# tuffy/libdvd-audio

Measured on AMD Instinct MI355X. Metric: decoded PCM Msamples/s (bit-exact) on 6ch/96k/24b MLP, higher is better.
Workload: dtype int32 (int64 accumulate)

## Files before the change

### libdvd-audio_amd/csrc/mlp_decode.h

```cpp
#pragma once
#include <hip/hip_runtime.h>
#if defined(__HIP_DEVICE_COMPILE__) && !defined(__gfx950__)
#error "mlp_decode.h is written for gfx950 (MI355X): hand-placed s_waitcnt encodings and gfx950 inline asm"
#endif
#include <stdint.h>
#include <type_traits>
#include "mlp_bounds.h"
#include "mlp_index.h"
#include "mlp_tables.h"

namespace mlp {

constexpr int DEC_THREADS = 128;
constexpr int DEC_WAVES = DEC_THREADS / 64;
constexpr int MAXCH = 8;
constexpr int MAXMAT = 6;
constexpr int RING_PLANES = 8;
constexpr int RING_DWORDS = RING_PLANES * 4;
constexpr int CHUNK_DWORDS = 16;
constexpr int OUT_ROWS = 4;
constexpr uint32_t YIELD_LONELY = 48;
#ifndef DVDA_HDR_GATE_TURNS
#define DVDA_HDR_GATE_TURNS 32
#endif
// ... 128 lines not shown
    const uint64_t *out_stride;
    uint32_t *seg_status;
    uint32_t *seg_rows;
    int32_t *iir_ws;
    uint32_t *mat_ws;
    uint32_t total_lanes;
    unsigned long long *dbg;
    int32_t *fir_ws;
    int32_t *fb;
    const int32_t *init_fir;
    DecodeSummary *summary;
    uint32_t interleaved;
    uint32_t wav_bits;
    uint32_t coop_min_seg;
    const uint32_t *hetero;
    const uint32_t *lane_seg;
    const uint32_t *cls;
    uint32_t only_S;
    uint32_t *seg_meta;
    uint32_t *yield_req;
    const uint32_t *seg_check;
    const uint32_t *list;
    uint32_t list_base, list_n;
    const uint32_t *list_n_ptr;
    const uint4 *plan;
    int32_t *res;
    uint32_t *brec;
    uint32_t *frec;
    WsCaps caps;
    uint32_t coop;
    struct CoopState *coop_state;
    struct CoopResult *coop_result;
    uint32_t coop_spare;
};

constexpr uint32_t COOP_MAX_SEG = 4096;
constexpr uint32_t COOP_MAX_AU = 32768;
__device__ __forceinline__ bool coop_takes(const DecodeArgs &a)
{
    if (a.coop)
        return a.coop == 64u;
    uint32_t n_seg = *a.n_seg_ptr;
    if (n_seg > a.max_seg)
        n_seg = a.max_seg;
    return n_seg <= COOP_MAX_SEG && a.seg_fbase[n_seg] <= COOP_MAX_AU;
}



__device__ __forceinline__ int32_t mask_q(int32_t x, uint32_t q)
{
    return (int32_t)((uint32_t)x & (0xFFFFFFFFu << q));
}
__device__ __forceinline__ uint32_t nib(uint32_t pack, uint32_t i) { return (pack >> (4 * i)) & 0xFu; }
__device__ __forceinline__ int32_t lo16(uint32_t v) { return (int32_t)(v << 16) >> 16; }
__device__ __forceinline__ int32_t hi16(uint32_t v) { return (int32_t)v >> 16; }

__device__ __forceinline__ int32_t huff_center(uint32_t codebook, uint32_t lb)
{
    if (codebook) {
        const int ss = (int)lb + 2 - (int)codebook;
        return 7 * (1 << lb) + (ss >= 0 ? (1 << ss) : 0);
    }
    const int ss = (int)lb - 1;
    return ss >= 0 ? (1 << ss) : 0;
}

__device__ __forceinline__ uint32_t be32(uint32_t v) { return __builtin_bswap32(v); }
template <int RD = RING_DWORDS>
__device__ __forceinline__ void ring_store16(uint32_t *dst, const uint4 &a, const uint4 &b, const uint4 &c,
                                             const uint4 &d, bool first_plane)
{
    const uint32_t a0 = be32(a.x);
    uint32_t *const e = dst - 15 * 64;
    if (first_plane)
        dst[-RD * 64] = a0;
    e[15 * 64] = a0;         e[14 * 64] = be32(a.y); e[13 * 64] = be32(a.z); e[12 * 64] = be32(a.w);
    e[11 * 64] = be32(b.x);  e[10 * 64] = be32(b.y); e[9 * 64] = be32(b.z);  e[8 * 64] = be32(b.w);
    e[7 * 64] = be32(c.x);   e[6 * 64] = be32(c.y);  e[5 * 64] = be32(c.z);  e[4 * 64] = be32(c.w);
    e[3 * 64] = be32(d.x);   e[2 * 64] = be32(d.y);  e[1 * 64] = be32(d.z);  e[0 * 64] = be32(d.w);
}

template <int RD>
__device__ __forceinline__ void ring_store4(uint32_t *dst, const uint4 &a, bool first_plane)
{
    const uint32_t a0 = be32(a.x);
    if (first_plane)
        dst[-RD * 64] = a0;
    dst[0] = a0;
    dst[-1 * 64] = be32(a.y);
    dst[-2 * 64] = be32(a.z);
    dst[-3 * 64] = be32(a.w);
}

__device__ __forceinline__ void ring_fill_sync(const uint4 *src, uint32_t *dst, bool first_plane)
{
    const uint4 a = src[0], b = src[1], c = src[2], d = src[3];
    ring_store16(dst, a, b, c, d, first_plane);
}

__device__ __attribute__((noinline)) int64_t iir_mac(const int32_t *ws, uint32_t stride)
{
    int64_t acc = 0;
    for (uint32_t j = 0; j < 8; j++)
        acc += (int64_t)ws[(size_t)j * stride] * (int64_t)ws[(size_t)(8 + j) * stride];
    return acc;
}

__device__ __attribute__((noinline)) void iir_push(int32_t *ws, uint32_t stride, int32_t v)
{
    for (int j = 7; j > 0; j--)
        ws[(size_t)(8 + j) * stride] = ws[(size_t)(8 + j - 1) * stride];
    ws[(size_t)8 * stride] = v;
}

template <int RD, int G>
struct BitReaderT {
    const uint4 *gsrc;
    uint32_t *ring;
    uint32_t max_chunk;
    uint32_t pos;
    uint32_t fillpos;
    uint32_t lo_valid;

    __device__ __forceinline__ uint32_t *slot(uint32_t d) const
    {
        return ring + ((RD - (d & (RD - 1))) << 6);
    }
    __device__ __forceinline__ uint64_t window() const
    {
        const uint32_t *p = ring + ((~(pos >> 5) & (RD - 1)) << 6);
        return ((uint64_t)p[64] << 32) | p[0];
    }
    __device__ __forceinline__ uint32_t window_lds() const
    {
        return (uint32_t)(uintptr_t)ring + ((~(pos >> 5) & (RD - 1)) << 8);
    }
    __device__ __forceinline__ int32_t ahead() const
    {
        return (int32_t)((fillpos << 5) - (pos & ~31u)) >> 5;
    }
    __device__ __forceinline__ void filled()
    {
        fillpos += G;
        if (fillpos - lo_valid > (uint32_t)RD)
            lo_valid = fillpos - RD;
    }
    __device__ __forceinline__ uint32_t fill_src() const
    {
        const uint32_t last = max_chunk + (uint32_t)(CHUNK_DWORDS - G);
        return fillpos < last ? fillpos : last;
    }
    __device__ __forceinline__ bool room() const { return ahead() <= (int32_t)(RD - G); }
    __device__ __forceinline__ void fill_sync()
    {
        if constexpr (G == CHUNK_DWORDS) {
            ring_fill_sync(gsrc + (fill_src() >> 2), slot(fillpos), (fillpos & (RD - 1)) == 0);
            filled();
        } else if constexpr (RD > 16) {
            uint4 q[4];
            const int32_t r = (RD - ahead()) >> 2;
            const int32_t n = r < 4 ? r : 4;
            const uint32_t end = max_chunk + (uint32_t)CHUNK_DWORDS;
#pragma unroll
            for (int g = 0; g < 4; g++) {
                const uint32_t e = fillpos + 4u * g + 4u;
                q[g] = gsrc[((e < end ? e : end) >> 2) - 1u];
            }
            __builtin_amdgcn_s_waitcnt(0x0F70);
            fill_commit(q, n);
        } else {
            uint4 q[4];
            const int32_t n = fill_issue(q);
            fill_commit(q, n);
        }
    }
    template <int MAXG = 4>
    __device__ __forceinline__ int32_t fill_issue(uint4 (&q)[MAXG]) const
    {
        static_assert(G == CHUNK_DWORDS || (G == 4 && (RD == 16 || RD == 32)),
                      "granule fills: the two small rings of a two-substream lane, or the 32-dword ring");
        int32_t n = room() ? (RD - ahead()) >> 2 : 0;
        if ((MAXG < 4 || RD > 16) && n > MAXG)
            n = MAXG;
#pragma unroll
        for (int g = 0; g < MAXG; g++)
            if (g < n) {
                const uint32_t f = fillpos + 4u * g, last = max_chunk + (uint32_t)(CHUNK_DWORDS - G);
                q[g] = gsrc[(f < last ? f : last) >> 2];
            }
        return n;
    }
    template <int MAXG = 4>
    __device__ __forceinline__ void fill_commit(const uint4 (&q)[MAXG], int32_t n)
    {
#pragma unroll
        for (int g = 0; g < MAXG; g++)
            if (g < n) {
                ring_store4<RD>(slot(fillpos), q[g], (fillpos & (RD - 1)) == 0);
                filled();
            }
    }
    __device__ __forceinline__ void ensure(uint32_t n)
    {
#if defined(DVDA_EXP_STAMP)
        const unsigned long long t0_ = clock64();
        bool any_ = false;
#endif
        while (__builtin_expect(__any(ahead() < (int32_t)n), 0)) {
            if (room())
                fill_sync();
#if defined(DVDA_EXP_STAMP)
            any_ = true;
#endif
        }
#if defined(DVDA_EXP_STAMP)
        if (any_) {
            fill_cyc += clock64() - t0_;
            fill_n++;
        }
#endif
    }
#if defined(DVDA_EXP_STAMP)
    unsigned long long fill_cyc = 0, fill_n = 0;
#endif
    __device__ __forceinline__ void seek_byte(uint64_t byte_pos)
    {
        const uint32_t t = (uint32_t)(byte_pos >> 2);
        if (!((int32_t)(t - lo_valid) >= 0 && (int32_t)(fillpos - t) > 0)) {
            fillpos = t & ~(uint32_t)(G - 1);
            lo_valid = fillpos;
        }
        pos = (uint32_t)byte_pos << 3;
    }
    __device__ __forceinline__ uint64_t tell_near(uint64_t ref_bits) const
    {
        return ref_bits + (uint64_t)(int64_t)(int32_t)(pos - (uint32_t)ref_bits);
    }
    __device__ __forceinline__ bool past(uint32_t end_bits_lo) const { return (int32_t)(pos - end_bits_lo) > 0; }
    __device__ __forceinline__ uint32_t peek32()
    {
        ensure(2);
        return (uint32_t)((window() << (pos & 31u)) >> 32);
    }
    __device__ __forceinline__ uint32_t read(uint32_t n)
    {
        const uint32_t top = peek32();
        pos += n;
        return n ? top >> (32 - n) : 0u;
    }
    __device__ __forceinline__ uint32_t read_resident(uint32_t n)
    {
        const uint32_t top = (uint32_t)((window() << (pos & 31u)) >> 32);
        pos += n;
        return (top >> 1) >> (31u - n);
    }
    __device__ __forceinline__ int32_t read_signed_resident(uint32_t n)
    {
        const uint32_t top = (uint32_t)((window() << (pos & 31u)) >> 32);
        pos += n;
        return n ? (int32_t)top >> ((32u - n) & 31u) : 0;
    }
    __device__ __forceinline__ int32_t read_signed(uint32_t n)
    {
        if (n == 0)
            return 0;
        const int32_t v = (int32_t)peek32() >> (32 - n);
        pos += n;
        return v;
    }
};

using BitReader = BitReaderT<RING_DWORDS, CHUNK_DWORDS>;
constexpr int DUO_RING = 16, DUO_GRAN = 4;

__host__ __device__ constexpr uint32_t hot_word(uint32_t cb, uint32_t lb, uint32_t q, uint32_t shift)
{
    return lb | (q << 5) | ((shift + q) << 10) |
           (cb ? ((7u - (8u >> cb)) << 16) | ((cb == 1 ? 9u : cb == 2 ? 7u : 6u) << 20) | ((4u - cb) << 24) |
                 ((28u + cb) << 26) | (1u << 31)
               : 0u);
// ... 11 lines not shown
    const uint32_t a = (top >> ((hw >> 26) & 31u)) + ((hw >> 16) & 0x307u);
    const uint32_t n = (uint32_t)__clz((int)((top & 0x3F800000u) | 0x00400000u));
    const uint32_t up = ((hw >> 20) & 0x10Fu) + n, dn = 0x108u - n;
    uint32_t d = 0x40000000u - (top & 0x7F800000u);
    asm("" : "+v"(d));
    uint32_t ms = (uint32_t)((int32_t)d >> 31);
    asm("" : "+v"(ms));
    uint32_t val = (up & ms) | (dn & ~ms);
    asm("" : "+v"(val));
    const uint32_t e = (n << 8) + val;
    uint32_t m = (uint32_t)((int32_t)top >> 31);
    asm("" : "+v"(m));
    return ((a & m) | (e & ~m)) & (uint32_t)((int32_t)hw >> 31);
}

__device__ __forceinline__ uint32_t huff_decode(uint32_t cb, uint32_t t)
{
    return huff_decode_top(t << 23, hot_word(cb, 0u, 0u, 0u));
}

struct SubPark {
    uint32_t flags, block_size, min_ch, max_ch, max_mat_ch, noise_shift, seed, matrix_len, bypass_mask, outch_pack,
             oshift_pack, qss_pack, nslots, iir_any, ss_end_bit, rows_left, blocks_in_frame, chk, gl, seg_lane;
    bool have_restart, seg_iir;
    uint32_t *brec, *brec_end, *brec_base;
};

template <int NS, bool PAIRED, bool GENERAL, bool ILV = false, bool PARSE = false, bool DUO = false, bool WAVO = false>
__global__ __launch_bounds__(DEC_THREADS, 2) void k_decode(DecodeArgs a)
{
    static_assert(!(GENERAL && PARSE), "one mode at a time");
    static_assert(!DUO || (!PAIRED && !GENERAL && NS == 6), "the two-substream lane is a one-lane fast-pass / parse instance");
    static_assert(GENERAL == PAIRED, "lane pairs are the sequential pass's layout, and its only one");
    constexpr uint32_t L = PAIRED ? 2u : 1u;
    if (!GENERAL && a.only_S && a.cls[a.only_S - 1u] == 0)
        return;
    if (!GENERAL && !PARSE && coop_takes(a))
        return;
    constexpr int THREADS = DEC_THREADS;
    constexpr int WAVES = THREADS / 64;
    constexpr int TP = 6;
    constexpr int PS = (ILV && !GENERAL && !PARSE && !DUO && !WAVO) ? 65 : 64;
    constexpr int RD = DUO ? DUO_RING : RING_DWORDS;
    constexpr bool WAVE_FILL = !DUO && !PAIRED;
    constexpr int RG = DUO ? DUO_GRAN : WAVE_FILL ? 4 : CHUNK_DWORDS;
    using Reader = BitReaderT<RD, RG>;
    __shared__ uint32_t s_ring[WAVES][DUO ? 2 : 1][RD + 1][64];
    __shared__ int32_t s_out[GENERAL ? 1 : WAVES][TP][OUT_ROWS][GENERAL ? 1 : PS];
    constexpr bool XCH = PAIRED;
    __shared__ int32_t s_xch[XCH ? WAVES : 1][MAXCH][XCH ? 64 : 1];
    __shared__ uint32_t s_nchained[WAVES];
    __shared__ uint16_t s_cold[WAVES][NS][64];

    if (threadIdx.x < WAVES)
        s_nchained[threadIdx.x] = 0;
    __syncthreads();

    const int lane = threadIdx.x & 63;
    const int wv = threadIdx.x >> 6;
    const uint32_t wg_id = blockIdx.x;
    const uint32_t gl0 = wg_id * THREADS + threadIdx.x;
    uint32_t n_seg = *a.n_seg_ptr;
    if (n_seg > a.max_seg)
        n_seg = a.max_seg;
    const uint32_t item = gl0 / L;
    uint32_t segi = item;
    bool active = segi < n_seg;
    if (!GENERAL && !PARSE && active && *a.hetero)
        segi = DVDA_AT(a.lane_seg, item, a.caps.max_seg, BT_LANE_SEG);
    if (!GENERAL && !PARSE && segi >= n_seg) {
        active = false;
        segi = n_seg;
    }
    if (GENERAL || PARSE) {
        active = item < a.list_n && (a.list_n_ptr == nullptr || item < *a.list_n_ptr) && (!PARSE || item < DVDA_AT(a.plan, n_seg, a.caps.max_seg + 1u, BT_PLAN).y);
        segi = 0;
        if (active) {
            const uint32_t e = DVDA_AT(a.list, a.list_base + item, GENERAL ? a.caps.max_streams : a.caps.max_seg, BT_LIST);
            segi = GENERAL ? DVDA_AT(a.streams, e, a.caps.max_streams, BT_STREAMS).first_seg : e;
            active = segi < n_seg;
        }
        if (!active)
            segi = n_seg;
    }

    SegRec sr;
    sr.off = sr.end = 0;
    sr.stream = 0;
    sr.nframes = 0;
    sr.flags = 0;
    sr.sync = 0;
    sr.ndrop = 0;
    sr.prev = 0xFFFFFFFFu;
    uint32_t fbase = 0, stream_sync = 0, stream_first = 0;
    if (active) {
        sr = DVDA_AT(a.seg, segi, a.caps.max_seg, BT_SEG);
        stream_first = DVDA_AT(a.streams, sr.stream, a.caps.max_streams, BT_STREAMS).first_seg;
        if (stream_first == 0xFFFFFFFFu) {
            active = false;
            stream_first = segi;
        } else {
            stream_sync = a.streams[sr.stream].sync;
            fbase = a.seg_fbase[segi] - DVDA_AT(a.seg_fbase, stream_first, a.caps.max_seg + 1u, BT_FBASE);
        }
    }
    const uint32_t S = (stream_sync >> 24) & 0xF;
    const uint32_t sub = DUO ? 1u : gl0 - item * L;
    uint32_t gl = segi * 2u + sub;
// ... 150 lines not shown
    constexpr bool CFU = !PARSE && !GENERAL && !DUO;
    constexpr int CFW = CFU ? 8 : 4;
    int32_t cf[NS][CFW];
    uint32_t pk[NS];
    int32_t sho[NS];
    uint32_t mreg[2][4];
    uint32_t mnoise[2] = {0, 0};
    constexpr bool MU = ILV && !PAIRED && !GENERAL && !PARSE && !DUO;
    int32_t mu[2][MU ? 8 : 1];
#pragma unroll
    for (int m = 0; m < 2; m++)
#pragma unroll
        for (int j = 0; j < (MU ? 8 : 1); j++)
            mu[m][j] = 0;
    constexpr bool PLACE = !GENERAL && !PARSE;
    constexpr bool MPK = DUO;
    uint32_t moff[2] = {0, 0};
    uint32_t mqm[2] = {0xFFFFFFFFu, 0xFFFFFFFFu};
    uint32_t mpk = 0;
    int32_t mk = 0;
    auto m_off = [&](int m) -> uint32_t { return MPK ? (mpk >> (11 * m)) & 0x7FFu : moff[m]; };
    auto m_qm = [&](int m) -> uint32_t { return MPK ? 0xFFFFFFFFu << ((mpk >> (22 + 4 * m)) & 0xFu) : mqm[m]; };
#pragma unroll
    for (int k = 0; k < NS; k++) {
#pragma unroll
        for (int j = 0; j < 4; j++)
            sp[k][j] = 0;
#pragma unroll
        for (int j = 0; j < CFW; j++)
            cf[k][j] = 0;
        pk[k] = hot_word(0u, 24u, 0u, 0u);
        s_cold[wv][k][lane] = (uint16_t)cold_word(0u, 0u, 0u, 0u);
        sho[k] = -(1 << 23);
    }
#pragma unroll
    for (int m = 0; m < 2; m++)
#pragma unroll
        for (int j = 0; j < 4; j++)
            mreg[m][j] = 0;
    if (GENERAL && resume_from_init) {
#pragma unroll
        for (int k = 0; k < NS; k++)
#pragma unroll
            for (int j = 0; j < 8; j++)
                st_set(k, j, a.init_fir[((size_t)sr.stream * 2 + sub) * 48 + k * 8 + j]);
    }
    uint32_t flags = 0xFF;
    uint32_t block_size = 8;
    uint32_t min_ch = 0, max_ch = 0, max_mat_ch = 0, noise_shift = 0, seed = 0;
    uint32_t matrix_len = 0, bypass_mask = 0, outch_pack = 0;
    uint32_t oshift_pack = 0, qss_pack = 0;
    uint32_t qss_A = 0, mmc_A = 0;
    uint32_t gate_turn = 0;
    auto no_restart_yet = [&]() -> uint32_t {
        if (GENERAL)
            return ST_ENVELOPE;
        const uint32_t first = a.streams[a.seg[segi].stream].first_seg;
        return segi != first ? ST_SEQ : ST_ENVELOPE;
    };
    constexpr bool HDR_GATE = !PAIRED && !GENERAL;
    const uint32_t gl_r = gl;
    uint32_t nslots = 0;
    bool have_restart = false;
    uint32_t iir_any = 0;
    bool seg_iir = false;

    uint64_t cur = sr.off;
    uint32_t ss_end_bit = 0;
    uint32_t rows_left = 0;
    bool in_frame = false;
    uint32_t frame_rows = 0;
    uint32_t blocks_in_frame = 0;
    uint32_t frames_done = 0;
    uint64_t row = row0;
    uint32_t rows_written = 0;
    uint32_t rows_done = 0;
    int32_t pq_s[OUT_ROWS] = {0, 0, 0, 0};
    uint32_t au_idx = 0;
    uint32_t drops_seen = 0;
    uint32_t dsub = sub;
    auto swap_sub = [&]() {
        auto sw = [](uint32_t &x, uint32_t &y) { const uint32_t t = x; x = y; y = t; };
        auto swb = [](bool &x, bool &y) { const bool t = x; x = y; y = t; };
        auto swp = [](uint32_t *&x, uint32_t *&y) { uint32_t *const t = x; x = y; y = t; };
        sw(rd.pos, rx.pos);
        sw(rd.fillpos, rx.fillpos);
        sw(rd.lo_valid, rx.lo_valid);
        swp(rd.ring, rx.ring);
        sw(flags, P0.flags);
        sw(block_size, P0.block_size);
        sw(min_ch, P0.min_ch);
        sw(max_ch, P0.max_ch);
        sw(max_mat_ch, P0.max_mat_ch);
        sw(noise_shift, P0.noise_shift);
        sw(seed, P0.seed);
        sw(matrix_len, P0.matrix_len);
        sw(bypass_mask, P0.bypass_mask);
        sw(outch_pack, P0.outch_pack);
        sw(oshift_pack, P0.oshift_pack);
        sw(qss_pack, P0.qss_pack);
        sw(nslots, P0.nslots);
        sw(iir_any, P0.iir_any);
        sw(ss_end_bit, P0.ss_end_bit);
        sw(rows_left, P0.rows_left);
        sw(blocks_in_frame, P0.blocks_in_frame);
        sw(chk, P0.chk);
// ... 18 lines not shown
            for (int c = 0; c < 6; c++)
                acc += (int64_t)ch[c] * (int64_t)((c & 1) ? hi16(mc[c >> 1]) : lo16(mc[c >> 1]));
            const uint32_t oc = nib(outch_pack, m);
            const int32_t nv = (int32_t)((uint32_t)mask_q((int32_t)(acc >> 14), nib(qss_A, oc)) +
                                         ((bypass_bits >> m) & 1u));
            uint32_t oce = on ? oc : 0xFFu;
            asm volatile("" : "+v"(oce));
            uint64_t hit[6];
#pragma unroll
            for (int c = 0; c < 6; c++) {
                hit[c] = __builtin_amdgcn_ballot_w64((uint32_t)c == oce);
                asm volatile("" : "+s"(hit[c]));
            }
#pragma unroll
            for (int c = 0; c < 6; c++) {
                int32_t keep = ch[c];
                asm("v_cndmask_b32_e64 %0, %0, %1, %2" : "+v"(keep) : "v"(nv), "s"(hit[c]));
                ch[c] = keep;
            }
        };
        if (__any(matrix_len > 0))
            one_matrix(mreg[0], mnoise[0], 0, matrix_len > 0);
        if (__any(matrix_len > 1))
            one_matrix(mreg[1], mnoise[1], 1, matrix_len > 1);
        if (GENERAL && __builtin_expect(__any(matrix_len > 2), 0)) {
            for (uint32_t m = 2; m < matrix_len; m++) {
                DVDA_COV(9);
                uint32_t mc[4];
#pragma unroll
                for (int j = 0; j < 4; j++)
                    mc[j] = a.mat_ws[(size_t)(m * 5 + j) * a.total_lanes + gl_r];
                one_matrix(mc, a.mat_ws[(size_t)(m * 5 + 4) * a.total_lanes + gl_r], m, true);
            }
        }
        if (__any(oshift_pack != 0)) {
#pragma unroll
            for (int c = 0; c < MAXCH; c++)
                if ((uint32_t)c <= mmc_A)
                    ch[c] = (int32_t)((uint32_t)ch[c] << nib(oshift_pack, c));
        }
    };

#if defined(DVDA_EXP_STAMP)
    unsigned long long stamp_acc[8] = {0, 0, 0, 0, 0, 0, 0, 0};
    unsigned long long stamp_t = clock64();
    unsigned long long hstamp_acc[6] = {0, 0, 0, 0, 0, 0};
    unsigned long long hfills = 0, hcount = 0;
    unsigned long long hstamp_t = 0;
#endif
    for (;;) {
        DVDA_STAMP(5);
        bool hdr_parsed = false;
        bool hdr_now = active && (rows_left == 0 || (DUO && P0.rows_left == 0));
        if (HDR_GATE && __builtin_expect(__any(hdr_now), 0)) {
            const uint64_t m_need = __ballot(hdr_now), m_act = __ballot(active);
            const bool go = m_need == m_act || (uint32_t)__popcll(m_need) >= HDR_GATE_LANES ||
                            (gate_turn & (HDR_GATE_TURNS - 1u)) == 0u;
            hdr_now = hdr_now && go;
        }
        gate_turn++;
        const bool hdr_wave = MU && __any(hdr_now);
        if constexpr (MU) {
            if (hdr_wave) {
#pragma unroll
                for (int m = 0; m < 2; m++) {
#pragma unroll
                    for (int j = 0; j < 3; j++)
                        mreg[m][j] = ((uint32_t)mu[m][MU ? 2 * j : 0] & 0xFFFFu) | ((uint32_t)mu[m][MU ? 2 * j + 1 : 0] << 16);
                    mnoise[m] = ((uint32_t)mu[m][MU ? 6 : 0] & 0xFFFFu) | ((uint32_t)mu[m][MU ? 7 : 0] << 16);
                }
            }
        }
        if (__builtin_expect(hdr_now, 0)) {
#if defined(DVDA_EXP_STAMP)
            hstamp_t = clock64();
            rd.fill_cyc = rd.fill_n = 0;
            if constexpr (DUO)
                rx.fill_cyc = rx.fill_n = 0;
#endif
            while (active && !in_frame) {
                if (frames_done == sr.nframes) {
                    if (GENERAL && a.fir_ws) {
#pragma unroll
                        for (int k = 0; k < NS; k++)
#pragma unroll
                            for (int j = 0; j < 8; j++)
                                a.fir_ws[(size_t)(k * 8 + j) * a.total_lanes + seg_lane] = st_get(k, j);
                    }
                    if (GENERAL || PARSE)
                        a.seg_meta[seg_lane] = min_ch | (max_ch << 4) | (1u << 8) | (seg_iir ? 1u << 9 : 0u);
                    if (PARSE && brec) {
#pragma unroll
                        for (int kk = 0; kk < 6; kk++)
                            brec[BREC_SLOT * kk] = 0xFFFFFFFFu;
                    }
                    if constexpr (DUO && PARSE) {
                        a.seg_meta[P0.seg_lane] = P0.min_ch | (P0.max_ch << 4) | (1u << 8) | (P0.seg_iir ? 1u << 9 : 0u);
                        if (P0.brec) {
#pragma unroll
                            for (int kk = 0; kk < 6; kk++)
                                P0.brec[BREC_SLOT * kk] = 0xFFFFFFFFu;
                        }
                    }
                    bool go_on = false;
                    if (GENERAL) {
                        atomicOr(&a.seg_status[segi], status | ((status & ~ST_INFO) ? 0u : ST_GENERAL));
                        if (is_last_sub)
                            a.seg_rows[segi] = rows_written;
                        uint32_t nxt = segi + 1;
                        while (nxt < n_seg && a.seg[nxt].stream == sr.stream && (a.seg[nxt].flags & SEG_DEAD))
                            nxt++;
// ... 36 lines not shown
                            cur = frame_end;
                            frames_done++;
                            drops_seen++;
                            continue;
                        }
                        rd.seek_byte(cur + 4);
                    }
                    uint32_t end_prev = 0, my_start = 0, my_end = 0, check0 = 0;
                    uint32_t end0 = 0;
                    bool bad = false;
                    for (uint32_t s = 0; s < S; s++) {
                        const uint32_t info = rd.read(16);
                        const uint32_t end = (info & 0xFFFu) * 2u;
                        if (info & 0x8000u)
                            rd.read(16);
                        if (s == 0) {
                            check0 = (info >> 13) & 1u;
                            end0 = end;
                        }
                        if (end < end_prev)
                            bad = true;
                        if (s == sub) {
                            my_start = end_prev;
                            my_end = end;
                        }
                        end_prev = end;
                    }
                    const uint64_t data0 = rd.tell_near(cur * 8u) >> 3;
                    const uint64_t ss_lo = data0 + my_start;
                    const uint64_t ss_hi = data0 + my_end;
                    if (bad || data0 + end_prev > frame_end || (check0 && my_end - my_start < 2) ||
                        (DUO && check0 && end0 < 2)) {
                        status |= ST_EOF;
                        active = false;
                    } else {
                        const uint64_t data_hi = check0 ? ss_hi - 2 : ss_hi;
                        ss_end_bit = (uint32_t)data_hi << 3;
                        rd.seek_byte(ss_lo);
                        if constexpr (DUO) {
                            P0.ss_end_bit = (uint32_t)(data0 + end0 - (check0 ? 2u : 0u)) << 3;
                            rx.seek_byte(data0);
                            P0.blocks_in_frame = 0;
                        }
                        in_frame = true;
                        frame_rows = 0;
                        blocks_in_frame = 0;
                        cur = frame_end;
                    }
                }
            }
            DVDA_HSTAMP(0);
            if (!GENERAL && !PARSE && active && frames_done < 2 && (frames_done | blocks_in_frame) != 0 &&
                (__hip_atomic_load(&a.yield_req[segi], __ATOMIC_RELAXED, __HIP_MEMORY_SCOPE_AGENT) ||
                 __hip_atomic_load(&s_nchained[wv], __ATOMIC_RELAXED, __HIP_MEMORY_SCOPE_WORKGROUP) >= YIELD_LONELY)) {
                status |= ST_YIELD;
                active = false;
            }
            bool probe = false;
#pragma nounroll
            for (uint32_t pass = DUO ? 0u : 1u; pass < 2u; pass++) {
                bool me = active;
                bool first0 = false;
                if constexpr (DUO) {
                    me = active && (pass == 0u ? P0.rows_left == 0u : rows_left == 0u);
                    if (!__any(me))
                        continue;
                    if (pass == 0u && me) {
                        swap_sub();
                        first0 = frames_done == 0u && blocks_in_frame == 0u;
                    }
                }
            if (me) {
                const bool mat_mine = !(DUO && dsub == 0u);
                bool ok = true;
                uint32_t err = ST_PARAMS;
                bool matrix_class_change = false;
                bool hdr_restart = false;
                uint32_t chg_mask = 0;
                bool seq_needed = false;
                if (rd.read(1)) {
                    rd.ensure(HDR_BLOCK);
                    const bool restart = rd.read_resident(1) != 0;
                    hdr_restart = restart;
                    if (restart) {
                        rd.ensure(HDR_RESTART);
                        const uint32_t h0 = rd.read_resident(14);
                        rd.read_resident(16);
                        min_ch = rd.read_resident(4);
                        max_ch = rd.read_resident(4);
                        max_mat_ch = rd.read_resident(4);
                        noise_shift = rd.read_resident(4);
                        seed = rd.read_resident(23);
                        rd.read_resident(19);
                        rd.read_resident(9);
                        rd.read_resident(16);
                        if (h0 != (0x18F5u << 1) || max_ch < min_ch || max_mat_ch < max_ch) {
                            ok = false;
                            err = ST_RESTART;
                        } else if (max_mat_ch >= 6u || max_ch - min_ch >= 6u || (!PAIRED && !DUO && min_ch != 0)) {
                            ok = false;
                            err = ST_ENVELOPE;
                        } else {
                            for (uint32_t c = 0; c <= max_mat_ch; c++)
                                if (rd.read_resident(6) > max_mat_ch) {
                                    ok = false;
                                    err = ST_RESTART;
                                }
// ... 329 lines not shown
                        }
                    }
                }
                DVDA_HSTAMP(3);
                if (!have_restart && ok) {
                    ok = false;
                    err = no_restart_yet();
                }
                hdr_parsed = true;
                if (PARSE && iir_any)
                    seg_iir = true;
                if (PARSE && ok && chg_mask) {
#pragma unroll
                    for (int kk = 0; kk < 6; kk++) {
                        brec[BREC_SLOT * kk] = rows_done;
                        brec[BREC_SLOT * kk + 1] = (chg_mask >> kk) & 1u;
                    }
                    brec += BREC_STRIDE;
                }
                if (PARSE && ok && (seq_needed || (hdr_restart && blocks_in_frame))) {
                    status |= ST_SEQ;
                    active = false;
                }
                if (mat_mine) {
                    qss_A = qss_pack;
                    mmc_A = max_mat_ch;
                    if constexpr (PLACE) {
                        mpk = 0;
#pragma unroll
                        for (int m = 0; m < 2; m++) {
                            const uint32_t oc = nib(outch_pack, m);
                            const uint32_t off = oc * ((ILV && ilv_direct) ? (uint32_t)PS : (uint32_t)(OUT_ROWS * PS));
                            if constexpr (MPK) {
                                mpk |= (off << (11 * m)) | (nib(qss_pack, oc) << (22 + 4 * m));
                            } else {
                                moff[m] = off;
                                mqm[m] = 0xFFFFFFFFu << nib(qss_pack, oc);
                            }
                        }
                    }
                }
                const uint32_t cold_ml = matrix_len;
                if (matrix_class_change)
                    status |= ST_MIDFRAME;
                if (!ok) {
                    status |= err;
                    active = false;
                } else if (PARSE && !active) {
                } else if (!GENERAL && !PARSE && (iir_any != 0 || cold_ml > 2)) {
                    status |= ST_COLD;
                    active = false;
                } else if (!GENERAL && !PARSE && (status & ST_CHAINED)) {
                    active = false;
                    if (!(DUO && probe))
                        atomicAdd(&s_nchained[wv], 1u);
                    if (sr.prev != 0xFFFFFFFFu)
                        __hip_atomic_store(&DVDA_AT(a.yield_req, sr.prev, a.caps.max_seg, BT_YIELD), 1u, __ATOMIC_RELAXED, __HIP_MEMORY_SCOPE_AGENT);
                } else {
                    rows_left = block_size;
                    blocks_in_frame++;
                    if (!GENERAL && !PARSE && frames_done < 2 &&
                        __hip_atomic_load(&s_nchained[wv], __ATOMIC_RELAXED, __HIP_MEMORY_SCOPE_WORKGROUP) >= YIELD_LONELY) {
                        status |= ST_YIELD;
                        active = false;
                    }
                }
            }
                if constexpr (DUO) {
                    if (pass == 0u && me)
                        swap_sub();
                    if (!PARSE && pass == 0u && me && !active && first0 && !(status & ~ST_INFO)) {
                        probe = true;
                        active = true;
                    }
                    if (pass == 1u && probe)
                        active = false;
                }
            }
            if constexpr (DUO) {
                if (active && have_restart && P0.have_restart && (P0.min_ch != 0u || min_ch != P0.max_ch + 1u)) {
                    status |= PARSE ? ST_SEQ : ST_COLD;
                    active = false;
                }
            }
        }
        if constexpr (MU) {
            if (hdr_wave) {
#pragma unroll
                for (int m = 0; m < 2; m++) {
#pragma unroll
                    for (int j = 0; j < 3; j++) {
                        mu[m][MU ? 2 * j : 0] = lo16(mreg[m][j]);
                        mu[m][MU ? 2 * j + 1 : 0] = hi16(mreg[m][j]);
                    }
                    mu[m][MU ? 6 : 0] = lo16(mnoise[m]);
                    mu[m][MU ? 7 : 0] = hi16(mnoise[m]);
                }
            }
        }
        if (hdr_now) {
            DVDA_HSTAMP(4);
#if defined(DVDA_EXP_STAMP)
            hstamp_acc[5] += rd.fill_cyc + (DUO ? rx.fill_cyc : 0ull);
            hfills += rd.fill_n + (DUO ? rx.fill_n : 0ull);
            hcount++;
#endif
        }
        if (!__any(active))
            break;
        DVDA_STAMP(0);

        if (active) {
            if constexpr (DUO) {
                while (__builtin_expect(__any(rd.ahead() < 8 || rx.ahead() < 8), 0)) {
                    DVDA_COV(14);
                    uint4 q[1];
                    asm volatile("" : "=v"(q[0].x), "=v"(q[0].y), "=v"(q[0].z), "=v"(q[0].w));
                    const int32_t n0 = rx.template fill_issue<1>(q);
                    rx.template fill_commit<1>(q, n0);
                    const int32_t n1 = rd.template fill_issue<1>(q);
                    rd.template fill_commit<1>(q, n1);
                }
            } else {
            if (rd.ahead() < 12)
                DVDA_COV(14);
            rd.ensure(12);
            }
        }
        DVDA_STAMP(7);
        constexpr int32_t FILL_TURN = 16;
        const bool pf = !WAVE_FILL && active && rd.room();
        const bool pfx = DUO && active && rx.room();
        int32_t fn = 0;
        uint4 p0, p1, p2, p3;
        asm volatile("" : "=v"(p0.x), "=v"(p0.y), "=v"(p0.z), "=v"(p0.w), "=v"(p1.x), "=v"(p1.y), "=v"(p1.z), "=v"(p1.w),
                          "=v"(p2.x), "=v"(p2.y), "=v"(p2.z), "=v"(p2.w), "=v"(p3.x), "=v"(p3.y), "=v"(p3.z), "=v"(p3.w));
        bool flush = false;
        const uint32_t frames_before = frames_done;
        uint64_t flush_row = 0;
        if constexpr (DUO) {
            if (pfx)
                p0 = rx.gsrc[rx.fill_src() >> 2];
            if (pf)
                p1 = rd.gsrc[rd.fill_src() >> 2];
        } else if constexpr (WAVE_FILL) {
            if (__any(active && rd.ahead() <= FILL_TURN)) {
                const int32_t r = (RD - rd.ahead()) >> 2;
                fn = active ? (r < 4 ? r : 4) : 0;
                const uint32_t end = rd.max_chunk + (uint32_t)CHUNK_DWORDS;
                const uint32_t last = end - 4u * (uint32_t)fn;
                const uint4 *src = rd.gsrc + ((rd.fillpos < last ? rd.fillpos : last) >> 2);
                if (fn > 0)
                    p0 = src[0];
                if (fn > 1)
                    p1 = src[1];
                if (fn > 2)
                    p2 = src[2];
                if (fn > 3)
                    p3 = src[3];
            }
        } else {
        if (pf) {
            const uint32_t c = rd.fillpos < rd.max_chunk ? rd.fillpos : rd.max_chunk;
            const uint4 *src = rd.gsrc + (c >> 2);
            p0 = src[0];
            p1 = src[1];
            p2 = src[2];
            p3 = src[3];
        }
        }
        DVDA_STAMP(1);

        uint32_t bypass_bits = 0;
        int32_t val[NS];
        auto row_head_any = [&]() {
            if (__any(bypass_mask != 0)) {
                const uint32_t cnt = (uint32_t)__popc(bypass_mask);
                const uint32_t field = rd.read_resident(cnt);
                const uint32_t b0 = bypass_mask & 1u, b1 = (bypass_mask >> 1) & 1u;
                bypass_bits = (b0 & (field >> ((cnt - 1u) & 31u))) | ((b1 & (field >> ((cnt - 1u - b0) & 31u))) << 1);
                if ((GENERAL || PARSE) && __builtin_expect(__any((bypass_mask >> 2) != 0), 0)) {
                    if (bypass_mask >> 2)
                        DVDA_COV(10);
                    uint32_t rank = b0 + b1;
#pragma unroll
                    for (int m = 2; m < MAXMAT; m++) {
                        const uint32_t bit = (bypass_mask >> m) & 1u;
                        bypass_bits |= (bit & (field >> ((cnt - 1u - rank) & 31u))) << m;
                        rank += bit;
                    }
                }
            }
            if constexpr (DUO)
                rx.pos += (uint32_t)__popc(P0.bypass_mask);
            uint32_t cpos = DUO ? rx.pos : rd.pos;
            uint32_t cbase = (uint32_t)(uintptr_t)(DUO ? rx.ring : rd.ring) + (uint32_t)((RD - 1) << 8);
            auto cur_window_lds = [&]() -> uint32_t { return cbase - ((cpos << 3) & (uint32_t)((RD - 1) << 8)); };
            uint64_t win = DUO ? rx.window() : rd.window();
            const uint32_t n_sub0 = DUO ? P0.max_ch + 1u : 0u;
            uint32_t msb_or = 0;
            const bool wave_iir = GENERAL && __any(iir_any != 0);
#pragma unroll
            for (int k = 0; k < NS; k++) {
                const bool in = DUO ? (uint32_t)k <= max_ch : (uint32_t)k < nslots;
                if (k > 0)
                    asm volatile("s_waitcnt lgkmcnt(0)" : "+v"(win));
                if constexpr (DUO) {
                    if (k > 0) {
                        const bool sw = (uint32_t)k == n_sub0;
                        if (__any(sw)) {
                            if (sw) {
                                rx.pos = cpos;
                                cpos = rd.pos;
                                cbase = (uint32_t)(uintptr_t)rd.ring + (uint32_t)((RD - 1) << 8);
                                win = rd.window();
                            }
                        }
                    }
                }
                val[k] = 0;
                if (k >= 2 && !__any(in))
                    continue;
                if (in) {
                const uint32_t hw = pk[k];
                const uint32_t lb = hw & 31u;
                const uint32_t ofs = cpos & 31u;
                const uint32_t top = (uint32_t)((win << ofs) >> 32);
                const uint32_t e = huff_decode_top(top, hw);
                const uint32_t msb = e & 0xFFu;
// ... 371 lines not shown
        int32_t ch[MAXCH];
        const bool in_row = active && (!HDR_GATE || (rows_left != 0 && (!DUO || P0.rows_left != 0)));
        if (in_row) {
            row_head_any();
            if (PAIRED) {
                const int slot0 = lane & ~1;
                int32_t(*X)[XCH ? 64 : 1] = s_xch[XCH ? wv : 0];
#pragma unroll
                for (int k = 0; k < NS; k++)
                    if ((uint32_t)k < nslots && min_ch + k < MAXCH)
                        X[min_ch + k][XCH ? slot0 : 0] = val[k];
                __builtin_amdgcn_fence(__ATOMIC_RELEASE, "wavefront");
                __builtin_amdgcn_wave_barrier();
                __builtin_amdgcn_fence(__ATOMIC_ACQUIRE, "wavefront");
#pragma unroll
                for (int c = 0; c < MAXCH; c++)
                    ch[c] = X[c][XCH ? slot0 : 0];
            } else {
#pragma unroll
                for (int c = 0; c < MAXCH; c++)
                    ch[c] = c < NS ? val[c < NS ? c : 0] : 0;
            }
            row_tail(ch);
            if constexpr (PLACE)
                flush = owner && !no_room && (rows_done & (OUT_ROWS - 1)) == 0;
        }
        if constexpr (GENERAL) {
            const int ended = frames_done != frames_before ? 1 : 0;
            const int other = __shfl_xor(ended, 1, 64);
            if (S == 2u && active && ended != other) {
                status |= ST_ENVELOPE;
                active = false;
            }
        }
        DVDA_STAMP(3);

#if defined(DVDA_EXP_STAMP)
        {
            asm volatile("s_waitcnt vmcnt(0)" ::: "memory");
            DVDA_STAMP(6);
        }
#endif
        __builtin_amdgcn_s_waitcnt(0x0F70);
        if constexpr (DUO) {
            if (pfx) {
                ring_store4<RD>(rx.slot(rx.fillpos), p0, (rx.fillpos & (RD - 1)) == 0);
                rx.filled();
            }
            if (pf) {
                ring_store4<RD>(rd.slot(rd.fillpos), p1, (rd.fillpos & (RD - 1)) == 0);
                rd.filled();
            }
        } else if constexpr (WAVE_FILL) {
            if (__any(fn > 0)) {
                const uint32_t f = rd.fillpos;
                if (fn > 0) {
                    ring_store4<RD>(rd.slot(f), p0, (f & (RD - 1)) == 0);
                    if (fn > 1) {
                        ring_store4<RD>(rd.slot(f + 4u), p1, ((f + 4u) & (RD - 1)) == 0);
                        if (fn > 2) {
                            ring_store4<RD>(rd.slot(f + 8u), p2, ((f + 8u) & (RD - 1)) == 0);
                            if (fn > 3)
                                ring_store4<RD>(rd.slot(f + 12u), p3, ((f + 12u) & (RD - 1)) == 0);
                        }
                    }
                    rd.fillpos = f + 4u * (uint32_t)fn;
                    if (rd.fillpos - rd.lo_valid > (uint32_t)RD)
                        rd.lo_valid = rd.fillpos - RD;
                }
            }
        } else {
        if (pf) {
            ring_store16(rd.slot(rd.fillpos), p0, p1, p2, p3, (rd.fillpos & (RING_DWORDS - 1)) == 0);
            rd.filled();
        }
        }
        auto out_row = [&]() -> uint64_t { return PLACE ? row0 + rows_done - (uint64_t)OUT_ROWS : flush_row; };
        bool coop_out = false;
        if constexpr (ILV && !GENERAL && !PARSE) {
            if (!WAVO && ilv_direct && a.wav_bits == 0u && a.coop_min_seg && n_seg >= a.coop_min_seg)
                coop_out = __ballot(flush) == ~0ull;
        }
        if (coop_out) {
            const uint64_t doff = out_base + out_row() * 6u;
            const bool off32 = !__any((doff >> 32) != 0);
            const uint32_t d_lo = (uint32_t)doff, d_hi = (uint32_t)(doff >> 32);
            const int32_t *const T0 = &s_out[GENERAL ? 0 : wv][0][0][0];
            const uint32_t l6 = ((uint32_t)lane * 43691u) >> 18;
            const uint32_t pc = (uint32_t)lane - l6 * 6u;
            const int32_t *const Tl6 = T0 + pc * (4 * PS) + l6;
            const bool l60 = lane < 60;
            if (__builtin_expect(off32, 1)) {
                uint32_t bo[7];
#pragma unroll
                for (uint32_t it7 = 0; it7 < 7u; it7++)
                    bo[it7] = (uint32_t)__shfl((int)d_lo, (int)(l6 + 10u * it7), 64);
                int32_t *const ob = a.pcm + pc * 4u;
                if (l60) {
                    const uint32_t ti = pc * (4u * PS) + l6;
                    auto piece = [&](uint32_t k, int32_t(&q)[4]) {
                        uint32_t tk = ti;
                        asm volatile("" : "+v"(tk));
#pragma unroll
                        for (uint32_t j = 0; j < 4u; j++)
                            q[j] = T0[tk + 10u * k + j * PS];
                    };
                    int32_t v[4][4];
#pragma unroll
                    for (uint32_t k = 0; k < 4u; k++)
                        piece(k, v[k]);
#pragma unroll
                    for (uint32_t k = 0; k < 4u; k++)
                        DVDA_STORE_V4_COOP(ob + bo[k], v[k][0], v[k][1], v[k][2], v[k][3]);
                    const bool last = lane < 24;
#pragma unroll
                    for (uint32_t k = 0; k < 2u; k++)
                        piece(4u + k, v[k]);
                    if (last)
                        piece(6u, v[2]);
#pragma unroll
                    for (uint32_t k = 0; k < 2u; k++)
                        DVDA_STORE_V4_COOP(ob + bo[4u + k], v[k][0], v[k][1], v[k][2], v[k][3]);
                    if (last)
                        DVDA_STORE_V4_COOP(ob + bo[6], v[2][0], v[2][1], v[2][2], v[2][3]);
                }
            } else {
#pragma unroll
            for (uint32_t it7 = 0; it7 < 7u; it7++) {
                const uint32_t o = l6 + 10u * it7;
                const uint32_t b_lo = (uint32_t)__shfl((int)d_lo, (int)o, 64);
                const uint64_t eo = b_lo | (uint64_t)(uint32_t)__shfl((int)d_hi, (int)o, 64) << 32;
                if (l60 && (it7 < 6u || o < 64u)) {
                    int32_t *const od = a.pcm + eo + pc * 4u;
                    const int32_t *const Tp = Tl6 + 10u * it7;
                    DVDA_STORE_V4_COOP(od, Tp[0], Tp[PS], Tp[2 * PS], Tp[3 * PS]);
                }
            }
            }
        }
        if (!GENERAL && !PARSE && ILV && flush && !coop_out) {
            const int32_t *Tl = &s_out[GENERAL ? 0 : wv][0][0][GENERAL ? 0 : lane];
            int32_t *dst = a.pcm + out_base + out_row() * nch_out;
            constexpr bool WAV_ELSEWHERE = !PAIRED && !WAVO && !DUO;
            if (WAVO || (!WAV_ELSEWHERE && __builtin_expect(a.wav_bits != 0, 0))) {
                const uint32_t nb = a.wav_bits >> 3;
                uint32_t *wd = reinterpret_cast<uint32_t *>(a.pcm + out_base) + (out_row() * nch_out * nb >> 2);
                if (ilv_direct && a.wav_bits == 24u) {
                    uint32_t d[18];
#pragma unroll
                    for (int g = 0; g < 6; g++) {
                        const int32_t o[4] = {Tl[(4 * g) * PS], Tl[(4 * g + 1) * PS], Tl[(4 * g + 2) * PS], Tl[(4 * g + 3) * PS]};
                        uint32_t t[3];
                        wav_pack4(o, 24u, t);
                        d[3 * g] = t[0];
                        d[3 * g + 1] = t[1];
                        d[3 * g + 2] = t[2];
                    }
#pragma unroll
                    for (int v = 0; v < 4; v++)
                        DVDA_STORE_V4_AT(wd, 16 * v, (int)d[4 * v], (int)d[4 * v + 1], (int)d[4 * v + 2], (int)d[4 * v + 3]);
                    DVDA_STORE_V2_AT(wd, 64, d[16], d[17]);
                } else {
                    uint32_t fi = 0, fw = 0;
                    for (uint32_t v = 0; v < nch_out; v++) {
                        int32_t o[4];
#pragma unroll
                        for (int j = 0; j < 4; j++) {
                            o[j] = ilv_direct ? Tl[(4 * v + j) * PS] : Tl[(nib(wave_inv, fw) * OUT_ROWS + fi) * PS];
                            fw++;
                            if (fw == nch_out) {
                                fw = 0;
                                fi++;
                            }
                        }
                        uint32_t d[3];
                        wav_pack4(o, a.wav_bits, d);
                        wd[nb * v] = d[0];
// ... 286 lines not shown
```

Measured before the change: 265,800.

## Micro-tune wave-fill ring stores, chained counting, and coop output addressing

Makes several unrelated micro-optimisations. Ring slot offsets for wave fills are now computed from a precomputed byte base, with a compile-time check that this matches slot() and first_plane, and the lo_valid clamp moves from every fill into seek_byte. In DUO mode the per-wave chained count is taken from a ballot popcount instead of shared-memory atomics. The cooperative output path now uses ds_bpermute and explicit LDS-address-space pointers to cut shuffle and address arithmetic. The gains are small and spread across the kernel, and moving the lo_valid update could be wrong if any other path depends on it.

```diff
diff --git a/libdvd-audio_amd/csrc/mlp_decode.h b/libdvd-audio_amd/csrc/mlp_decode.h
--- a/libdvd-audio_amd/csrc/mlp_decode.h
+++ b/libdvd-audio_amd/csrc/mlp_decode.h
@@ -204,6 +204,8 @@
 {
     return (int32_t)((uint32_t)x & (0xFFFFFFFFu << q));
 }
+__device__ __forceinline__ uint64_t wave_mask(bool p) { return __builtin_amdgcn_ballot_w64(p); }
+__device__ __forceinline__ bool wave_any(bool p) { return wave_mask(p) != 0ull; }
 __device__ __forceinline__ uint32_t nib(uint32_t pack, uint32_t i) { return (pack >> (4 * i)) & 0xFu; }
 __device__ __forceinline__ int32_t lo16(uint32_t v) { return (int32_t)(v << 16) >> 16; }
 __device__ __forceinline__ int32_t hi16(uint32_t v) { return (int32_t)v >> 16; }
@@ -245,6 +247,40 @@
     dst[-3 * 64] = be32(a.w);
 }
 
+template <int RD>
+__host__ __device__ constexpr uint32_t ring_turn_off(uint32_t f8, uint32_t g)
+{
+    return (f8 + g * 0x400u) & ((uint32_t)(RD - 1) << 8);
+}
+template <int RD>
+__host__ __device__ constexpr uint32_t ring_slot_index(uint32_t d)
+{
+    return (uint32_t)(RD - (d & (RD - 1))) << 6;
+}
+template <int RD>
+__host__ __device__ constexpr bool ring_turn_off_ok()
+{
+    const uint32_t bases[] = {0u, (uint32_t)RD, 0x00FFFFE0u, 0x7FFFFFE0u, 0xFFFFFFC0u, 0xFFFFFFE0u};
+    for (uint32_t b : bases)
+        for (uint32_t k = 0; k < (uint32_t)RD; k += 4u)
+            for (uint32_t fn = 0; fn <= 4u; fn++) {
+                const uint32_t f = b + k, f8 = f << 8;
+                for (uint32_t g = 0; g < fn; g++) {
+                    const uint32_t d = f + 4u * g, off = ring_turn_off<RD>(f8, g);
+                    if ((off & 0xFFu) != 0u || off > (uint32_t)(RD - 4) * 256u)
+                        return false;
+                    if ((uint32_t)RD * 64u - (off >> 2) != ring_slot_index<RD>(d))
+                        return false;
+                    if ((off == 0u) != ((d & (uint32_t)(RD - 1)) == 0u))
+                        return false;
+                }
+                if (((f + 4u * fn) & 3u) != 0u)
+                    return false;
+            }
+    return true;
+}
+static_assert(ring_turn_off_ok<RING_DWORDS>(), "ring_turn_off disagrees with BitReaderT::slot() / first_plane");
+
 __device__ __forceinline__ void ring_fill_sync(const uint4 *src, uint32_t *dst, bool first_plane)
 {
     const uint4 a = src[0], b = src[1], c = src[2], d = src[3];
@@ -277,7 +313,7 @@
 
     __device__ __forceinline__ uint32_t *slot(uint32_t d) const
     {
-        return ring + ((RD - (d & (RD - 1))) << 6);
+        return ring + ring_slot_index<RD>(d);
     }
     __device__ __forceinline__ uint64_t window() const
     {
@@ -379,6 +415,10 @@
     __device__ __forceinline__ void seek_byte(uint64_t byte_pos)
     {
         const uint32_t t = (uint32_t)(byte_pos >> 2);
+        if constexpr (G == 4 && RD > 16) {
+            if (fillpos - lo_valid > (uint32_t)RD)
+                lo_valid = fillpos - RD;
+        }
         if (!((int32_t)(t - lo_valid) >= 0 && (int32_t)(fillpos - t) > 0)) {
             fillpos = t & ~(uint32_t)(G - 1);
             lo_valid = fillpos;
@@ -496,8 +536,10 @@
     __shared__ uint32_t s_nchained[WAVES];
     __shared__ uint16_t s_cold[WAVES][NS][64];
 
-    if (threadIdx.x < WAVES)
-        s_nchained[threadIdx.x] = 0;
+    if constexpr (!DUO) {
+        if (threadIdx.x < WAVES)
+            s_nchained[threadIdx.x] = 0;
+    }
     __syncthreads();
 
     const int lane = threadIdx.x & 63;
@@ -754,6 +796,13 @@
     uint32_t oshift_pack = 0, qss_pack = 0;
     uint32_t qss_A = 0, mmc_A = 0;
     uint32_t gate_turn = 0;
+    uint32_t wave_chained = 0;
+    auto n_chained = [&]() -> uint32_t {
+        if constexpr (DUO)
+            return wave_chained;
+        else
+            return __hip_atomic_load(&s_nchained[wv], __ATOMIC_RELAXED, __HIP_MEMORY_SCOPE_WORKGROUP);
+    };
     auto no_restart_yet = [&]() -> uint32_t {
         if (GENERAL)
             return ST_ENVELOPE;
@@ -878,11 +927,14 @@
         DVDA_STAMP(5);
         bool hdr_parsed = false;
         bool hdr_now = active && (rows_left == 0 || (DUO && P0.rows_left == 0));
-        if (HDR_GATE && __builtin_expect(__any(hdr_now), 0)) {
-            const uint64_t m_need = __ballot(hdr_now), m_act = __ballot(active);
+        const uint64_t m_need = DUO ? __ballot(hdr_now) : wave_mask(active) & wave_mask(rows_left == 0);
+        if (HDR_GATE && __builtin_expect(m_need != 0ull, 0)) {
+            const uint64_t m_act = __ballot(active);
             const bool go = m_need == m_act || (uint32_t)__popcll(m_need) >= HDR_GATE_LANES ||
                             (gate_turn & (HDR_GATE_TURNS - 1u)) == 0u;
             hdr_now = hdr_now && go;
+            if constexpr (DUO && !PARSE)
+                wave_chained = (uint32_t)__popcll(~m_act & wave_mask((status & (ST_CHAINED | ST_COLD)) == ST_CHAINED));
         }
         gate_turn++;
         const bool hdr_wave = MU && __any(hdr_now);
@@ -1025,7 +1077,7 @@
             DVDA_HSTAMP(0);
             if (!GENERAL && !PARSE && active && frames_done < 2 && (frames_done | blocks_in_frame) != 0 &&
                 (__hip_atomic_load(&a.yield_req[segi], __ATOMIC_RELAXED, __HIP_MEMORY_SCOPE_AGENT) ||
-                 __hip_atomic_load(&s_nchained[wv], __ATOMIC_RELAXED, __HIP_MEMORY_SCOPE_WORKGROUP) >= YIELD_LONELY)) {
+                 n_chained() >= YIELD_LONELY)) {
                 status |= ST_YIELD;
                 active = false;
             }
@@ -1461,7 +1513,7 @@
                     active = false;
                 } else if (!GENERAL && !PARSE && (status & ST_CHAINED)) {
                     active = false;
-                    if (!(DUO && probe))
+                    if constexpr (!DUO)
                         atomicAdd(&s_nchained[wv], 1u);
                     if (sr.prev != 0xFFFFFFFFu)
                         __hip_atomic_store(&DVDA_AT(a.yield_req, sr.prev, a.caps.max_seg, BT_YIELD), 1u, __ATOMIC_RELAXED, __HIP_MEMORY_SCOPE_AGENT);
@@ -1469,7 +1521,7 @@
                     rows_left = block_size;
                     blocks_in_frame++;
                     if (!GENERAL && !PARSE && frames_done < 2 &&
-                        __hip_atomic_load(&s_nchained[wv], __ATOMIC_RELAXED, __HIP_MEMORY_SCOPE_WORKGROUP) >= YIELD_LONELY) {
+                        n_chained() >= YIELD_LONELY) {
                         status |= ST_YIELD;
                         active = false;
                     }
@@ -1553,8 +1605,9 @@
             if (pf)
                 p1 = rd.gsrc[rd.fill_src() >> 2];
         } else if constexpr (WAVE_FILL) {
-            if (__any(active && rd.ahead() <= FILL_TURN)) {
-                const int32_t r = (RD - rd.ahead()) >> 2;
+            const int32_t ahead_bits = (int32_t)((rd.fillpos << 5) - (rd.pos & ~31u));
+            if (wave_any(active && ahead_bits <= FILL_TURN * 32)) {
+                const int32_t r = (RD * 32 - ahead_bits) >> 7;
                 fn = active ? (r < 4 ? r : 4) : 0;
                 const uint32_t end = rd.max_chunk + (uint32_t)CHUNK_DWORDS;
                 const uint32_t last = end - 4u * (uint32_t)fn;
@@ -1583,7 +1636,7 @@
         uint32_t bypass_bits = 0;
         int32_t val[NS];
         auto row_head_any = [&]() {
-            if (__any(bypass_mask != 0)) {
+            if (wave_any(bypass_mask != 0)) {
                 const uint32_t cnt = (uint32_t)__popc(bypass_mask);
                 const uint32_t field = rd.read_resident(cnt);
                 const uint32_t b0 = bypass_mask & 1u, b1 = (bypass_mask >> 1) & 1u;
@@ -2061,21 +2114,24 @@
                 rd.filled();
             }
         } else if constexpr (WAVE_FILL) {
-            if (__any(fn > 0)) {
-                const uint32_t f = rd.fillpos;
+            if (wave_any(fn > 0)) {
+                const uint32_t f = rd.fillpos, f8 = f << 8;
+                char *const top = reinterpret_cast<char *>(rd.ring) + RD * 256;
+                auto put = [&](uint32_t g, const uint4 &p) {
+                    const uint32_t off = ring_turn_off<RD>(f8, g);
+                    ring_store4<RD>(reinterpret_cast<uint32_t *>(top - off), p, off == 0u);
+                };
                 if (fn > 0) {
-                    ring_store4<RD>(rd.slot(f), p0, (f & (RD - 1)) == 0);
+                    put(0u, p0);
                     if (fn > 1) {
-                        ring_store4<RD>(rd.slot(f + 4u), p1, ((f + 4u) & (RD - 1)) == 0);
+                        put(1u, p1);
                         if (fn > 2) {
-                            ring_store4<RD>(rd.slot(f + 8u), p2, ((f + 8u) & (RD - 1)) == 0);
+                            put(2u, p2);
                             if (fn > 3)
-                                ring_store4<RD>(rd.slot(f + 12u), p3, ((f + 12u) & (RD - 1)) == 0);
+                                put(3u, p3);
                         }
                     }
                     rd.fillpos = f + 4u * (uint32_t)fn;
-                    if (rd.fillpos - rd.lo_valid > (uint32_t)RD)
-                        rd.lo_valid = rd.fillpos - RD;
                 }
             }
         } else {
@@ -2088,11 +2144,14 @@
         bool coop_out = false;
         if constexpr (ILV && !GENERAL && !PARSE) {
             if (!WAVO && ilv_direct && a.wav_bits == 0u && a.coop_min_seg && n_seg >= a.coop_min_seg)
-                coop_out = __ballot(flush) == ~0ull;
+                coop_out = wave_mask(flush) == ~0ull;
         }
         if (coop_out) {
-            const uint64_t doff = out_base + out_row() * 6u;
-            const bool off32 = !__any((doff >> 32) != 0);
+            const uint64_t orow = out_row();
+            uint64_t orow2 = orow << 1;
+            asm("" : "+v"(orow2));
+            const uint64_t doff = out_base + (orow << 2) + orow2;
+            const bool off32 = !wave_any((doff >> 32) != 0);
             const uint32_t d_lo = (uint32_t)doff, d_hi = (uint32_t)(doff >> 32);
             const int32_t *const T0 = &s_out[GENERAL ? 0 : wv][0][0][0];
             const uint32_t l6 = ((uint32_t)lane * 43691u) >> 18;
@@ -2101,18 +2160,23 @@
             const bool l60 = lane < 60;
             if (__builtin_expect(off32, 1)) {
                 uint32_t bo[7];
+                const uint32_t l6x4 = l6 << 2;
 #pragma unroll
                 for (uint32_t it7 = 0; it7 < 7u; it7++)
-                    bo[it7] = (uint32_t)__shfl((int)d_lo, (int)(l6 + 10u * it7), 64);
-                int32_t *const ob = a.pcm + pc * 4u;
+                    bo[it7] = (uint32_t)__builtin_amdgcn_ds_bpermute((int)(l6x4 + 40u * it7), (int)d_lo);
+                char *const ob = reinterpret_cast<char *>(a.pcm + pc * 4u);
+                uint32_t four = 4u;
+                asm("" : "+s"(four));
+                auto at = [&](uint32_t k) { return reinterpret_cast<int32_t *>(ob + (uint64_t)bo[k] * four); };
                 if (l60) {
-                    const uint32_t ti = pc * (4u * PS) + l6;
+                    typedef const int32_t __attribute__((address_space(3))) *lds_i32p;
+                    uint32_t ta = (uint32_t)(uintptr_t)(T0 + pc * (4u * PS) + l6);
                     auto piece = [&](uint32_t k, int32_t(&q)[4]) {
-                        uint32_t tk = ti;
-                        asm volatile("" : "+v"(tk));
+                        asm volatile("" : "+v"(ta));
+                        const lds_i32p Tk = (lds_i32p)ta;
 #pragma unroll
                         for (uint32_t j = 0; j < 4u; j++)
-                            q[j] = T0[tk + 10u * k + j * PS];
+                            q[j] = Tk[10u * k + j * PS];
                     };
                     int32_t v[4][4];
 #pragma unroll
@@ -2120,7 +2184,7 @@
                         piece(k, v[k]);
 #pragma unroll
                     for (uint32_t k = 0; k < 4u; k++)
-                        DVDA_STORE_V4_COOP(ob + bo[k], v[k][0], v[k][1], v[k][2], v[k][3]);
+                        DVDA_STORE_V4_COOP(at(k), v[k][0], v[k][1], v[k][2], v[k][3]);
                     const bool last = lane < 24;
 #pragma unroll
                     for (uint32_t k = 0; k < 2u; k++)
@@ -2129,9 +2193,9 @@
                         piece(6u, v[2]);
 #pragma unroll
                     for (uint32_t k = 0; k < 2u; k++)
-                        DVDA_STORE_V4_COOP(ob + bo[4u + k], v[k][0], v[k][1], v[k][2], v[k][3]);
+                        DVDA_STORE_V4_COOP(at(4u + k), v[k][0], v[k][1], v[k][2], v[k][3]);
                     if (last)
-                        DVDA_STORE_V4_COOP(ob + bo[6], v[2][0], v[2][1], v[2][2], v[2][3]);
+                        DVDA_STORE_V4_COOP(at(6u), v[2][0], v[2][1], v[2][2], v[2][3]);
                 }
             } else {
 #pragma unroll
```

New measurement: 269,300 (median of 6 runs). 1.01x the previous value.
